# rbuler/multimodal-isic

Hardware: AMD Instinct MI355X
Metric: bags/sec (train step) @ 64x224x224 patches/bag (higher is better)
Workload: dtype bf16; 1 GPU; ISIC-shaped attention-MIL: 256 bags x 64x224x224 patches + 128-d radiomics, ResNet-18 encoder, bf16 (BASELINE.json configs[1]); patches_per_bag=64, patch=3x224x224, radiomics_dim=128, parallelism=dp1

## Files before the change

### multimodal-isic_amd/csrc/conv_stem.hip

```cpp
#include <type_traits>

#include "common.h"
#include "pool_grad.h"

namespace {

constexpr int TH = 8, TW = 16;
constexpr int PR = 2 * TH + 5, PC = 40;
constexpr int PROW = PC * 8;
constexpr int WROW = 7 * 64 + 16;
constexpr int CPAD = 72;
constexpr int YROW = 128 + 32;
constexpr int STEM_DW_ELEMS = 64 * 7 * 7 * 3;
constexpr int STEM_WGRAD_BLOCKS = 512;
constexpr int STEM_FWD_BLOCKS = 768;

struct StemArgs {
  const unsigned short* in;
  const unsigned short* w;
  unsigned short* out;
  const unsigned short* dy;
  float* dw;
  double* stat_sum;
  double* stat_sumsq;
  int stat_slots;
  int N, Hin, Win, Hout, Wout, tiles_h, tiles_w, total_tiles;
};

constexpr int PATCH_PER_THREAD = (PR * PC + 255) / 256;
__device__ __forceinline__ void fetch_patch(u32x2 (&r)[PATCH_PER_THREAD], const StemArgs& a, int tile, int tid) {
  const int n = tile / (a.tiles_h * a.tiles_w);
  const int t2 = tile - n * (a.tiles_h * a.tiles_w);
  const int oy0 = (t2 / a.tiles_w) * TH, ox0 = (t2 % a.tiles_w) * TW;
#pragma unroll
  for (int u = 0; u < PATCH_PER_THREAD; ++u) {
    const int idx = tid + 256 * u;
    const int pr = idx / PC, pc = idx - pr * PC;
    const int hi = 2 * oy0 - 3 + pr, wi = 2 * ox0 - 3 + pc;
    u32x2 v = {0u, 0u};
    if (tile < a.total_tiles && idx < PR * PC && hi >= 0 && hi < a.Hin && wi >= 0 && wi < a.Win)
      v = *reinterpret_cast<const u32x2*>(a.in + (((size_t)n * a.Hin + hi) * a.Win + wi) * 4);
    r[u] = v;
  }
}
__device__ __forceinline__ void commit_patch(unsigned char* Ps, const u32x2 (&r)[PATCH_PER_THREAD], int tid) {
#pragma unroll
  for (int u = 0; u < PATCH_PER_THREAD; ++u) {
    const int idx = tid + 256 * u;
    if (idx < PR * PC) {
      const int pr = idx / PC, pc = idx - pr * PC;
      *reinterpret_cast<u32x2*>(Ps + pr * PROW + pc * 8) = r[u];
    }
  }
}

__global__ __launch_bounds__(256) void conv_stem_fwd_kernel(StemArgs a) {
  static_assert(TH * TW * CPAD * 2 >= PR * PROW, "the C tile overlays the patch");
  __shared__ __attribute__((aligned(16))) unsigned char smem[64 * WROW + TH * TW * CPAD * 2];
  unsigned char* Ws = smem;
  unsigned char* Ps = smem + 64 * WROW;
  unsigned short* Cs = reinterpret_cast<unsigned short*>(smem + 64 * WROW);
  const int tid = threadIdx.x, lane = tid & 63, wave = tid >> 6;
  const int fi = lane & 15, fg = lane >> 4;

  for (int idx = tid; idx < 64 * 28; idx += 256) {
    const int co = idx / 28, ch = idx - co * 28;
    *reinterpret_cast<u32x4*>(Ws + co * WROW + ch * 16) = *reinterpret_cast<const u32x4*>(a.w + co * 224 + ch * 8);
  }

  u32x2 pre[PATCH_PER_THREAD];
  fetch_patch(pre, a, blockIdx.x, tid);
  float st_s[4][4], st_q[4][4];
#pragma unroll
  for (int j = 0; j < 4; ++j)
#pragma unroll
    for (int r = 0; r < 4; ++r) { st_s[j][r] = 0.f; st_q[j][r] = 0.f; }
  for (int tile = blockIdx.x; tile < a.total_tiles; tile += gridDim.x) {
    const int n = tile / (a.tiles_h * a.tiles_w);
    const int t2 = tile - n * (a.tiles_h * a.tiles_w);
    const int oy0 = (t2 / a.tiles_w) * TH, ox0 = (t2 % a.tiles_w) * TW;
    lds_barrier();
    commit_patch(Ps, pre, tid);
    lds_barrier();
    fetch_patch(pre, a, tile + gridDim.x, tid);

    f32x4 acc[2][4];
#pragma unroll
    for (int i = 0; i < 2; ++i)
#pragma unroll
      for (int j = 0; j < 4; ++j) acc[i][j] = (f32x4){0.f, 0.f, 0.f, 0.f};
#pragma unroll
    for (int kh = 0; kh < 7; ++kh) {
      bf16x8 af[2], bfr[4];
#pragma unroll
      for (int i = 0; i < 2; ++i) {
        const int oyl = wave * 2 + i;
        af[i] = *reinterpret_cast<const bf16x8*>(Ps + (2 * oyl + kh) * PROW + (2 * fi + 2 * fg) * 8);
      }
#pragma unroll
      for (int j = 0; j < 4; ++j)
        bfr[j] = *reinterpret_cast<const bf16x8*>(Ws + (j * 16 + fi) * WROW + kh * 64 + fg * 16);
#pragma unroll
      for (int i = 0; i < 2; ++i)
#pragma unroll
        for (int j = 0; j < 4; ++j)
          acc[i][j] = __builtin_amdgcn_mfma_f32_16x16x32_bf16(bfr[j], af[i], acc[i][j], 0, 0, 0);
    }
    lds_barrier();
#pragma unroll
    for (int i = 0; i < 2; ++i)
#pragma unroll
      for (int j = 0; j < 4; ++j) {
        const int p = (wave * 2 + i) * 16 + fi;
        u32x2 v;
        v[0] = (unsigned)f32_to_bf16_bits(acc[i][j][0]) | ((unsigned)f32_to_bf16_bits(acc[i][j][1]) << 16);
        v[1] = (unsigned)f32_to_bf16_bits(acc[i][j][2]) | ((unsigned)f32_to_bf16_bits(acc[i][j][3]) << 16);
        *reinterpret_cast<u32x2*>(Cs + p * CPAD + j * 16 + fg * 4) = v;
        if (a.stat_sum) {
          const bool in = (oy0 + wave * 2 + i < a.Hout) && (ox0 + fi < a.Wout);
          const float r0 = in ? __uint_as_float(v[0] << 16) : 0.f, r1 = in ? __uint_as_float(v[0] & 0xFFFF0000u) : 0.f;
          const float r2 = in ? __uint_as_float(v[1] << 16) : 0.f, r3 = in ? __uint_as_float(v[1] & 0xFFFF0000u) : 0.f;
          st_s[j][0] += r0; st_q[j][0] += r0 * r0;
          st_s[j][1] += r1; st_q[j][1] += r1 * r1;
          st_s[j][2] += r2; st_q[j][2] += r2 * r2;
          st_s[j][3] += r3; st_q[j][3] += r3 * r3;
        }
      }
    lds_barrier();
    for (int idx = tid; idx < TH * TW * 8; idx += 256) {
      const int p = idx >> 3, ch = idx & 7;
      const int oy = oy0 + (p >> 4), ox = ox0 + (p & 15);
      if (oy < a.Hout && ox < a.Wout)
        __builtin_nontemporal_store(*reinterpret_cast<const u32x4*>(Cs + p * CPAD + ch * 8),
                                    reinterpret_cast<u32x4*>(a.out + (((size_t)n * a.Hout + oy) * a.Wout + ox) * 64 + ch * 8));
    }
  }
  if (a.stat_sum) {
    __shared__ float stat_red[2][4][64];
    lds_barrier();
#pragma unroll
    for (int j = 0; j < 4; ++j)
#pragma unroll
      for (int r = 0; r < 4; ++r) {
        float sv = st_s[j][r], qv = st_q[j][r];
#pragma unroll
        for (int o = 8; o > 0; o >>= 1) { sv += __shfl_xor(sv, o, 16); qv += __shfl_xor(qv, o, 16); }
        if (fi == 0) { stat_red[0][wave][j * 16 + fg * 4 + r] = sv; stat_red[1][wave][j * 16 + fg * 4 + r] = qv; }
      }
    lds_barrier();
    if (tid < 128) {
      const int c = tid & 63, w = tid >> 6;
      const float t = (stat_red[w][0][c] + stat_red[w][1][c]) + (stat_red[w][2][c] + stat_red[w][3][c]);
      const size_t slot = (size_t)(blockIdx.x % a.stat_slots) * 64 + c;
      atomicAdd((w == 0 ? a.stat_sum : a.stat_sumsq) + slot, (double)t);
    }
  }
}

__global__ __launch_bounds__(256) void conv_stem_wgrad_kernel(StemArgs a) {
  __shared__ __attribute__((aligned(16))) unsigned char smem[PR * PROW + TH * TW * YROW];
  unsigned char* Ps = smem;
  unsigned char* Ys = smem + PR * PROW;
  const int tid = threadIdx.x, lane = tid & 63, wave = tid >> 6;
  const int fg = lane >> 4, fi = lane & 15, fq = fi >> 2, fp = fi & 3;
  typedef __attribute__((address_space(3))) s16x4* lds_s16x4;

  f32x4 acc[4][4];
#pragma unroll
  for (int i = 0; i < 4; ++i)
#pragma unroll
    for (int j = 0; j < 4; ++j) acc[i][j] = (f32x4){0.f, 0.f, 0.f, 0.f};

  u32x2 pre[PATCH_PER_THREAD];
  u32x4 prey[4];
  auto fetch_dy = [&](int tile) {
    const int n = tile / (a.tiles_h * a.tiles_w);
    const int t2 = tile - n * (a.tiles_h * a.tiles_w);
    const int oy0 = (t2 / a.tiles_w) * TH, ox0 = (t2 % a.tiles_w) * TW;
#pragma unroll
    for (int u = 0; u < 4; ++u) {
      const int idx = tid + 256 * u;
      const int p = idx >> 3, ch = idx & 7;
      const int oy = oy0 + (p >> 4), ox = ox0 + (p & 15);
      u32x4 v = {0u, 0u, 0u, 0u};
      if (tile < a.total_tiles && oy < a.Hout && ox < a.Wout)
        v = *reinterpret_cast<const u32x4*>(a.dy + (((size_t)n * a.Hout + oy) * a.Wout + ox) * 64 + ch * 8);
      prey[u] = v;
    }
  };
  fetch_patch(pre, a, blockIdx.x, tid);
  fetch_dy(blockIdx.x);
  for (int tile = blockIdx.x; tile < a.total_tiles; tile += gridDim.x) {
    lds_barrier();
    commit_patch(Ps, pre, tid);
#pragma unroll
    for (int u = 0; u < 4; ++u) {
      const int idx = tid + 256 * u;
      *reinterpret_cast<u32x4*>(Ys + (idx >> 3) * YROW + (idx & 7) * 16) = prey[u];
    }
    lds_barrier();
    fetch_patch(pre, a, tile + gridDim.x, tid);
    fetch_dy(tile + gridDim.x);
#pragma unroll
    for (int ks = 0; ks < 4; ++ks) {
      const int k1 = ks * 32 + 8 * fg + fq, k2 = k1 + 4;
      bf16x8 af[4], bfr[4];
#pragma unroll
      for (int i = 0; i < 4; ++i) {
        const s16x4 lo = __builtin_amdgcn_ds_read_tr16_b64_v4i16((lds_s16x4)(Ys + k1 * YROW + (i * 16 + 4 * fp) * 2));
        const s16x4 hi = __builtin_amdgcn_ds_read_tr16_b64_v4i16((lds_s16x4)(Ys + k2 * YROW + (i * 16 + 4 * fp) * 2));
        s16x8_t t; t.lo = lo; t.hi = hi;
        af[i] = __builtin_bit_cast(bf16x8, t);
      }
#pragma unroll
      for (int j = 0; j < 4; ++j) {
        const int nt = wave + 4 * j;
        const int kh = nt >> 1, half = nt & 1;
        const int khc = kh > 6 ? 6 : kh;
        const unsigned char* p1 = Ps + (2 * (k1 >> 4) + khc) * PROW + (2 * (k1 & 15) + half * 4 + fp) * 8;
        const unsigned char* p2 = Ps + (2 * (k2 >> 4) + khc) * PROW + (2 * (k2 & 15) + half * 4 + fp) * 8;
        const s16x4 lo = __builtin_amdgcn_ds_read_tr16_b64_v4i16((lds_s16x4)p1);
        const s16x4 hi = __builtin_amdgcn_ds_read_tr16_b64_v4i16((lds_s16x4)p2);
        s16x8_t t; t.lo = lo; t.hi = hi;
        bfr[j] = __builtin_bit_cast(bf16x8, t);
      }
#pragma unroll
      for (int i = 0; i < 4; ++i)
#pragma unroll
        for (int j = 0; j < 4; ++j)
          acc[i][j] = __builtin_amdgcn_mfma_f32_16x16x32_bf16(af[i], bfr[j], acc[i][j], 0, 0, 0);
    }
  }
#pragma unroll
  for (int i = 0; i < 4; ++i)
#pragma unroll
    for (int j = 0; j < 4; ++j) {
      const int nt = wave + 4 * j;
      if (nt >= 14) continue;
      const int kh = nt >> 1, kw = (nt & 1) * 4 + (fi >> 2), c = fi & 3;
      if (kw >= 7 || c >= 3) continue;
#pragma unroll
      for (int r = 0; r < 4; ++r) {
        const int co = i * 16 + fg * 4 + r;
        a.dw[(size_t)blockIdx.x * STEM_DW_ELEMS + ((co * 7 + kh) * 7 + kw) * 3 + c] = acc[i][j][r];
      }
    }
}

struct StemBnArgs {
  StemArgs s;
  const unsigned short* y0;
  const unsigned char* argmax;
  const unsigned short* gp;
  const float* mean; const float* rstd; const float* gamma; const float* scale; const float* shift;
  const double* dgamma; const double* dbeta;
  float* dgamma_f32; float* dbeta_f32;
  int Hp, Wp;
};

__global__ __launch_bounds__(256, 2) void conv_stem_wgrad_bn_kernel(StemBnArgs b) {
  const StemArgs& a = b.s;
  __shared__ __attribute__((aligned(16))) unsigned char smem[PR * PROW + TH * TW * YROW];
  __shared__ __attribute__((aligned(16))) float cst[5][64];
  unsigned char* Ps = smem;
  unsigned char* Ys = smem + PR * PROW;
  const int tid = threadIdx.x, lane = tid & 63, wave = tid >> 6;
  const int fg = lane >> 4, fi = lane & 15, fq = fi >> 2, fp = fi & 3;
  typedef __attribute__((address_space(3))) s16x4* lds_s16x4;
  const isic_pool::PoolGeom geom{a.Hout, a.Wout, 64, b.Hp, b.Wp};

  if (tid < 64) {
    const float inv_rows = 1.f / (float)((int64_t)a.N * a.Hout * a.Wout);
    const float rs = b.rstd[tid], mu = b.mean[tid], k1 = b.gamma[tid] * rs;
    const float k2 = (float)b.dbeta[tid] * inv_rows, k3 = (float)b.dgamma[tid] * inv_rows;
    cst[0][tid] = k1; cst[1][tid] = -k1 * k3 * rs; cst[2][tid] = k1 * (k3 * rs * mu - k2);
    cst[3][tid] = b.scale[tid]; cst[4][tid] = b.shift[tid];
    if (blockIdx.x == 0 && b.dgamma_f32) {
      b.dgamma_f32[tid] += (float)b.dgamma[tid];
      b.dbeta_f32[tid] += (float)b.dbeta[tid];
    }
  }

  f32x4 acc[4][4];
#pragma unroll
  for (int i = 0; i < 4; ++i)
#pragma unroll
    for (int j = 0; j < 4; ++j) acc[i][j] = (f32x4){0.f, 0.f, 0.f, 0.f};

  const int cg = tid & 7, bl = tid >> 3, al = bl >> 3, bw = bl & 7;
  u32x2 pre[PATCH_PER_THREAD];
  u32x4 xr[4];
  isic_pool::Windows win;
  auto fetch_dy = [&](int tile) {
    const int tc = tile < a.total_tiles ? tile : a.total_tiles - 1;
    const int n = tc / (a.tiles_h * a.tiles_w);
    const int t2 = tc - n * (a.tiles_h * a.tiles_w);
    const int oy0 = (t2 / a.tiles_w) * TH, ox0 = (t2 % a.tiles_w) * TW;
    const int ga = (oy0 >> 1) + al, gb = (ox0 >> 1) + bw;
#pragma unroll
    for (int p = 0; p < 4; ++p) {
      const int hi = min(2 * ga + (p >> 1), a.Hout - 1), wi = min(2 * gb + (p & 1), a.Wout - 1);
      xr[p] = *reinterpret_cast<const u32x4*>(b.y0 + (((size_t)n * a.Hout + hi) * a.Wout + wi) * 64 + cg * 8);
    }
    isic_pool::load_windows(win, b.argmax, b.gp, geom, n, min(ga, b.Hp - 1), min(gb, b.Wp - 1), cg);
  };
  auto commit_dy = [&](int tile) {
    const int n = tile / (a.tiles_h * a.tiles_w);
    const int t2 = tile - n * (a.tiles_h * a.tiles_w);
    const int oy0 = (t2 / a.tiles_w) * TH, ox0 = (t2 % a.tiles_w) * TW;
    const int ga = (oy0 >> 1) + al, gb = (ox0 >> 1) + bw;
    const bool inside = (oy0 + TH <= a.Hout) && (ox0 + TW <= a.Wout);
    auto half = [&](auto HC) {
      constexpr int H_ = decltype(HC)::value;
      float g[4][4];
      isic_pool::windows_to_grad4<H_>(win, geom, ga, gb, g);
      const int c0 = cg * 8 + H_ * 4;
      const f32x4 kA = *reinterpret_cast<const f32x4*>(&cst[0][c0]), kB = *reinterpret_cast<const f32x4*>(&cst[1][c0]);
      const f32x4 kD = *reinterpret_cast<const f32x4*>(&cst[2][c0]), sc = *reinterpret_cast<const f32x4*>(&cst[3][c0]);
      const f32x4 sh = *reinterpret_cast<const f32x4*>(&cst[4][c0]);
#pragma unroll
      for (int p = 0; p < 4; ++p) {
        const int oyl = 2 * al + (p >> 1), oxl = 2 * bw + (p & 1);
        const bool in = inside || ((oy0 + oyl < a.Hout) && (ox0 + oxl < a.Wout));
        const unsigned lo = xr[p][2 * H_], hi = xr[p][2 * H_ + 1];
        const float xv[4] = {__uint_as_float(lo << 16), __uint_as_float(lo & 0xFFFF0000u), __uint_as_float(hi << 16),
                             __uint_as_float(hi & 0xFFFF0000u)};
        float o[4];
#pragma unroll
        for (int j = 0; j < 4; ++j) {
          const float dz = (xv[j] * sc[j] + sh[j] > 0.f) ? g[p][j] : 0.f;
          o[j] = kA[j] * dz + (kB[j] * xv[j] + kD[j]);
          if (!inside) o[j] = in ? o[j] : 0.f;
        }
        u32x2 v;
        v[0] = (unsigned)f32_to_bf16_bits(o[0]) | ((unsigned)f32_to_bf16_bits(o[1]) << 16);
        v[1] = (unsigned)f32_to_bf16_bits(o[2]) | ((unsigned)f32_to_bf16_bits(o[3]) << 16);
        *reinterpret_cast<u32x2*>(Ys + (oyl * TW + oxl) * YROW + cg * 16 + H_ * 8) = v;
      }
    };
    half(std::integral_constant<int, 0>{});
    __builtin_amdgcn_sched_barrier(0);
    half(std::integral_constant<int, 1>{});
  };
  __syncthreads();
  fetch_patch(pre, a, blockIdx.x, tid);
  fetch_dy(blockIdx.x);
  for (int tile = blockIdx.x; tile < a.total_tiles; tile += gridDim.x) {
    lds_barrier();
    commit_patch(Ps, pre, tid);
    commit_dy(tile);
    lds_barrier();
    fetch_patch(pre, a, tile + gridDim.x, tid);
    fetch_dy(tile + gridDim.x);
#pragma unroll
    for (int ks = 0; ks < 4; ++ks) {
      const int k1 = ks * 32 + 8 * fg + fq, k2 = k1 + 4;
      bf16x8 af[4], bfr[4];
#pragma unroll
      for (int i = 0; i < 4; ++i) {
        const s16x4 lo = __builtin_amdgcn_ds_read_tr16_b64_v4i16((lds_s16x4)(Ys + k1 * YROW + (i * 16 + 4 * fp) * 2));
        const s16x4 hi = __builtin_amdgcn_ds_read_tr16_b64_v4i16((lds_s16x4)(Ys + k2 * YROW + (i * 16 + 4 * fp) * 2));
        s16x8_t t; t.lo = lo; t.hi = hi;
        af[i] = __builtin_bit_cast(bf16x8, t);
      }
#pragma unroll
      for (int j = 0; j < 4; ++j) {
        const int nt = wave + 4 * j;
        const int kh = nt >> 1, half = nt & 1;
        const int khc = kh > 6 ? 6 : kh;
        const unsigned char* p1 = Ps + (2 * (k1 >> 4) + khc) * PROW + (2 * (k1 & 15) + half * 4 + fp) * 8;
        const unsigned char* p2 = Ps + (2 * (k2 >> 4) + khc) * PROW + (2 * (k2 & 15) + half * 4 + fp) * 8;
        const s16x4 lo = __builtin_amdgcn_ds_read_tr16_b64_v4i16((lds_s16x4)p1);
        const s16x4 hi = __builtin_amdgcn_ds_read_tr16_b64_v4i16((lds_s16x4)p2);
        s16x8_t t; t.lo = lo; t.hi = hi;
        bfr[j] = __builtin_bit_cast(bf16x8, t);
      }
#pragma unroll
      for (int i = 0; i < 4; ++i)
#pragma unroll
        for (int j = 0; j < 4; ++j)
          acc[i][j] = __builtin_amdgcn_mfma_f32_16x16x32_bf16(af[i], bfr[j], acc[i][j], 0, 0, 0);
    }
  }
#pragma unroll
  for (int i = 0; i < 4; ++i)
#pragma unroll
    for (int j = 0; j < 4; ++j) {
      const int nt = wave + 4 * j;
      if (nt >= 14) continue;
      const int kh = nt >> 1, kw = (nt & 1) * 4 + (fi >> 2), c = fi & 3;
      if (kw >= 7 || c >= 3) continue;
#pragma unroll
      for (int r = 0; r < 4; ++r) {
        const int co = i * 16 + fg * 4 + r;
        a.dw[(size_t)blockIdx.x * STEM_DW_ELEMS + ((co * 7 + kh) * 7 + kw) * 3 + c] = acc[i][j][r];
      }
    }
}

__global__ __launch_bounds__(256) void stem_wgrad_reduce_kernel(const float* __restrict__ partial, float* __restrict__ dw,
                                                                 int nparts) {
  const int g = threadIdx.x & 15;
  const int e = blockIdx.x * 16 + (threadIdx.x >> 4);
  float v = 0.f;
  if (e < STEM_DW_ELEMS)
    for (int s = g; s < nparts; s += 16) v += partial[(size_t)s * STEM_DW_ELEMS + e];
#pragma unroll
  for (int o = 8; o > 0; o >>= 1) v += __shfl_xor(v, o, 16);
  if (e < STEM_DW_ELEMS && g == 0) dw[e] += v;
}

__global__ void stem_pack_kernel(const float* __restrict__ w, unsigned short* __restrict__ ws) {
  const int idx = blockIdx.x * blockDim.x + threadIdx.x;
  if (idx >= 64 * 7 * 8 * 4) return;
  const int c = idx & 3, kw = (idx >> 2) & 7, kh = (idx >> 5) % 7, co = idx / 224;
  float v = 0.f;
  if (c < 3 && kw < 7) v = w[((co * 7 + kh) * 7 + kw) * 3 + c];
  ws[idx] = f32_to_bf16_bits(v);
}

int stem_args(StemArgs& a, int N, int Hin, int Win, int Hout, int Wout) {
  if (Hout != (Hin + 6 - 7) / 2 + 1 || Wout != (Win + 6 - 7) / 2 + 1) return ISIC_ERR_BAD_ARG;
  a.N = N; a.Hin = Hin; a.Win = Win; a.Hout = Hout; a.Wout = Wout;
  a.tiles_h = ceil_div(Hout, TH); a.tiles_w = ceil_div(Wout, TW);
  const int64_t tt = (int64_t)N * a.tiles_h * a.tiles_w;
  if (tt > 0x7FFFFFFFLL) return ISIC_ERR_UNSUPPORTED;
  a.total_tiles = (int)tt;
  return ISIC_OK;
}

}

extern "C" {

int isic_conv_stem_fwd_bf16(const uint16_t* in_nhwc4, const uint16_t* w_stem, uint16_t* out, int N, int Hin, int Win,
                            int Hout, int Wout, void* stream) {
  return isic_conv_stem_fwd_stats_bf16(in_nhwc4, w_stem, out, N, Hin, Win, Hout, Wout, nullptr, nullptr, 0, stream);
}

int isic_conv_stem_fwd_stats_bf16(const uint16_t* in_nhwc4, const uint16_t* w_stem, uint16_t* out, int N, int Hin,
                                  int Win, int Hout, int Wout, double* stat_sum, double* stat_sumsq, int stat_slots,
                                  void* stream) {
  ISIC_CHECK_ARG(in_nhwc4 && w_stem && out && N > 0 && Hin > 0 && Win > 0);
  ISIC_CHECK_ARG((stat_sum == nullptr) == (stat_sumsq == nullptr));
  ISIC_CHECK_ARG(!stat_sum || stat_slots > 0);
  StemArgs a;
  a.stat_sum = stat_sum; a.stat_sumsq = stat_sumsq; a.stat_slots = stat_slots > 0 ? stat_slots : 1;
  a.in = in_nhwc4; a.w = w_stem; a.out = out; a.dy = nullptr; a.dw = nullptr;
  int rc = stem_args(a, N, Hin, Win, Hout, Wout);
  if (rc != ISIC_OK) return rc;
  const int grid = a.total_tiles < STEM_FWD_BLOCKS ? a.total_tiles : STEM_FWD_BLOCKS;
  hipLaunchKernelGGL(conv_stem_fwd_kernel, dim3(grid), dim3(256), 0, as_stream(stream), a);
  return isic_launch_status();
}

size_t isic_conv_stem_wgrad_workspace_bytes(void) { return (size_t)STEM_WGRAD_BLOCKS * STEM_DW_ELEMS * sizeof(float); }

int isic_conv_stem_wgrad_bf16(const uint16_t* in_nhwc4, const uint16_t* dy, float* dw, int N, int Hin, int Win,
                              int Hout, int Wout, void* workspace, size_t workspace_bytes, void* stream) {
  ISIC_CHECK_ARG(in_nhwc4 && dy && dw && workspace && N > 0 && Hin > 0 && Win > 0);
  if (workspace_bytes < isic_conv_stem_wgrad_workspace_bytes()) return ISIC_ERR_WORKSPACE;
  StemArgs a;
  a.stat_sum = nullptr; a.stat_sumsq = nullptr; a.stat_slots = 1;
  a.in = in_nhwc4; a.w = nullptr; a.out = nullptr; a.dy = dy; a.dw = reinterpret_cast<float*>(workspace);
  int rc = stem_args(a, N, Hin, Win, Hout, Wout);
  if (rc != ISIC_OK) return rc;
  const int grid = a.total_tiles < STEM_WGRAD_BLOCKS ? a.total_tiles : STEM_WGRAD_BLOCKS;
  hipLaunchKernelGGL(conv_stem_wgrad_kernel, dim3(grid), dim3(256), 0, as_stream(stream), a);
  hipLaunchKernelGGL(stem_wgrad_reduce_kernel, dim3(ceil_div(STEM_DW_ELEMS, 16)), dim3(256), 0, as_stream(stream),
                     reinterpret_cast<const float*>(workspace), dw, grid);
  return isic_launch_status();
}

int isic_conv_stem_wgrad_bn_pooled_bf16(const uint16_t* in_nhwc4, const uint16_t* y0, const uint8_t* argmax,
                                        const uint16_t* dy_pooled, const float* mean, const float* rstd,
                                        const float* gamma, const float* scale, const float* shift, const double* dgamma,
                                        const double* dbeta, float* dw, float* dgamma_f32, float* dbeta_f32, int N,
                                        int Hin, int Win, int Hout, int Wout, int Hp, int Wp, void* workspace,
                                        size_t workspace_bytes, void* stream) {
  ISIC_CHECK_ARG(in_nhwc4 && y0 && argmax && dy_pooled && mean && rstd && gamma && scale && shift && dgamma && dbeta && dw);
  ISIC_CHECK_ARG(workspace != nullptr);
  if (workspace_bytes < isic_conv_stem_wgrad_workspace_bytes()) return ISIC_ERR_WORKSPACE;
  ISIC_CHECK_ARG(N > 0 && Hin > 0 && Win > 0 && (dgamma_f32 == nullptr) == (dbeta_f32 == nullptr));
  ISIC_CHECK_ARG(Hp == (Hout + 2 - 3) / 2 + 1 && Wp == (Wout + 2 - 3) / 2 + 1);
  StemBnArgs b;
  StemArgs& a = b.s;
  a.stat_sum = nullptr; a.stat_sumsq = nullptr; a.stat_slots = 1;
  a.in = in_nhwc4; a.w = nullptr; a.out = nullptr; a.dy = nullptr; a.dw = reinterpret_cast<float*>(workspace);
  int rc = stem_args(a, N, Hin, Win, Hout, Wout);
  if (rc != ISIC_OK) return rc;
  b.y0 = y0; b.argmax = argmax; b.gp = dy_pooled; b.mean = mean; b.rstd = rstd; b.gamma = gamma; b.scale = scale;
  b.shift = shift; b.dgamma = dgamma; b.dbeta = dbeta; b.dgamma_f32 = dgamma_f32; b.dbeta_f32 = dbeta_f32;
  b.Hp = Hp; b.Wp = Wp;
  const int grid = a.total_tiles < STEM_WGRAD_BLOCKS ? a.total_tiles : STEM_WGRAD_BLOCKS;
  hipLaunchKernelGGL(conv_stem_wgrad_bn_kernel, dim3(grid), dim3(256), 0, as_stream(stream), b);
  hipLaunchKernelGGL(stem_wgrad_reduce_kernel, dim3(ceil_div(STEM_DW_ELEMS, 16)), dim3(256), 0, as_stream(stream),
                     reinterpret_cast<const float*>(workspace), dw, grid);
  return isic_launch_status();
}

int isic_conv_stem_pack_bf16(const float* w_krsc, uint16_t* w_stem, void* stream) {
  ISIC_CHECK_ARG(w_krsc && w_stem);
  hipLaunchKernelGGL(stem_pack_kernel, dim3(ceil_div(64 * 224, 256)), dim3(256), 0, as_stream(stream), w_krsc, w_stem);
  return isic_launch_status();
}

}
```

Baseline: 915.8 bags/s.

## Interleave next-tile prefetch with BN backward and inline maxpool grad routing

The fused stem wgrad+BN backward kernel now issues the next tile's patch, y0 and pool-window loads between the halves of the current tile's BN-backward commit, rather than after the LDS barrier. The goal is to hide global-load latency behind ALU work. Maxpool gradient routing is inlined with explicit argmax code selection and bf16 rounding. Blocks are also remapped so neighbouring block ids take strided tile ranges, with partial dw indexed to match. The added sched_barriers and live registers may raise register pressure at 2 waves/SIMD.

Result: faster. 928.1 bags/s (median of 6 runs) (+1.3%).

```diff
diff --git a/multimodal-isic_amd/csrc/conv_stem.hip b/multimodal-isic_amd/csrc/conv_stem.hip
--- a/multimodal-isic_amd/csrc/conv_stem.hip
+++ b/multimodal-isic_amd/csrc/conv_stem.hip
@@ -247,6 +247,21 @@
     }
 }
 
+typedef __attribute__((ext_vector_type(2))) float f32x2;
+typedef __attribute__((ext_vector_type(2))) __bf16 bf16x2;
+__device__ __forceinline__ unsigned pack_bf16x2(float lo, float hi) {
+  return __builtin_bit_cast(unsigned, __builtin_convertvector((f32x2){lo, hi}, bf16x2));
+}
+__device__ __forceinline__ float bn_bwd_value(float kA, float kB, float kD, float x, float dz) {
+#pragma clang fp contract(off)
+  return (kB * x + kD) + kA * dz;
+}
+__device__ __forceinline__ void round_bf16_pair(float& x, float& y) {
+  const unsigned v = pack_bf16x2(x, y);
+  x = __uint_as_float(v << 16);
+  y = __uint_as_float(v & 0xFFFF0000u);
+}
+
 struct StemBnArgs {
   StemArgs s;
   const unsigned short* y0;
@@ -287,33 +302,58 @@
 #pragma unroll
     for (int j = 0; j < 4; ++j) acc[i][j] = (f32x4){0.f, 0.f, 0.f, 0.f};
 
+  const int lb = gridDim.x % 8 == 0 ? (blockIdx.x % 8) * (gridDim.x / 8) + blockIdx.x / 8 : blockIdx.x;
   const int cg = tid & 7, bl = tid >> 3, al = bl >> 3, bw = bl & 7;
   u32x2 pre[PATCH_PER_THREAD];
   u32x4 xr[4];
   isic_pool::Windows win;
-  auto fetch_dy = [&](int tile) {
+  struct TileGeo { int n, oy0, ox0, ga, gb; };
+  auto geo = [&](int tile) {
     const int tc = tile < a.total_tiles ? tile : a.total_tiles - 1;
-    const int n = tc / (a.tiles_h * a.tiles_w);
-    const int t2 = tc - n * (a.tiles_h * a.tiles_w);
-    const int oy0 = (t2 / a.tiles_w) * TH, ox0 = (t2 % a.tiles_w) * TW;
-    const int ga = (oy0 >> 1) + al, gb = (ox0 >> 1) + bw;
-#pragma unroll
-    for (int p = 0; p < 4; ++p) {
-      const int hi = min(2 * ga + (p >> 1), a.Hout - 1), wi = min(2 * gb + (p & 1), a.Wout - 1);
-      xr[p] = *reinterpret_cast<const u32x4*>(b.y0 + (((size_t)n * a.Hout + hi) * a.Wout + wi) * 64 + cg * 8);
-    }
-    isic_pool::load_windows(win, b.argmax, b.gp, geom, n, min(ga, b.Hp - 1), min(gb, b.Wp - 1), cg);
+    TileGeo t;
+    t.n = tc / (a.tiles_h * a.tiles_w);
+    const int t2 = tc - t.n * (a.tiles_h * a.tiles_w);
+    t.oy0 = (t2 / a.tiles_w) * TH; t.ox0 = (t2 % a.tiles_w) * TW;
+    t.ga = (t.oy0 >> 1) + al; t.gb = (t.ox0 >> 1) + bw;
+    return t;
+  };
+  auto fetch_y0 = [&](const TileGeo& t, int p) {
+    const int hi = min(2 * t.ga + (p >> 1), a.Hout - 1), wi = min(2 * t.gb + (p & 1), a.Wout - 1);
+    xr[p] = *reinterpret_cast<const u32x4*>(b.y0 + (((size_t)t.n * a.Hout + hi) * a.Wout + wi) * 64 + cg * 8);
+  };
+  auto fetch_windows = [&](const TileGeo& t) {
+    isic_pool::load_windows(win, b.argmax, b.gp, geom, t.n, min(t.ga, b.Hp - 1), min(t.gb, b.Wp - 1), cg);
   };
   auto commit_dy = [&](int tile) {
-    const int n = tile / (a.tiles_h * a.tiles_w);
-    const int t2 = tile - n * (a.tiles_h * a.tiles_w);
-    const int oy0 = (t2 / a.tiles_w) * TH, ox0 = (t2 % a.tiles_w) * TW;
-    const int ga = (oy0 >> 1) + al, gb = (ox0 >> 1) + bw;
-    const bool inside = (oy0 + TH <= a.Hout) && (ox0 + TW <= a.Wout);
-    auto half = [&](auto HC) {
+    const TileGeo t = geo(tile), nx = geo(tile + gridDim.x);
+    const bool live01 = t.gb + 1 < b.Wp, live10 = t.ga + 1 < b.Hp, live11 = live01 && live10;
+    float dz[2][4][4];
+    auto route = [&](auto HC) {
       constexpr int H_ = decltype(HC)::value;
-      float g[4][4];
-      isic_pool::windows_to_grad4<H_>(win, geom, ga, gb, g);
+      const unsigned am[4] = {win.am[0][H_], live01 ? win.am[1][H_] : ~0u, live10 ? win.am[2][H_] : ~0u,
+                              live11 ? win.am[3][H_] : ~0u};
+#pragma unroll
+      for (int j = 0; j < 4; ++j) {
+        float g[4];
+#pragma unroll
+        for (int k = 0; k < 4; ++k) {
+          const unsigned w = win.g[k][2 * H_ + (j >> 1)];
+          g[k] = __uint_as_float((j & 1) ? (w & 0xFFFF0000u) : (w << 16));
+        }
+        g[0] = g[0] + 0.f;
+        auto sel = [&](int k, unsigned code) { return ((am[k] >> (8 * j)) & 0xFFu) == code ? g[k] : 0.f; };
+        dz[H_][0][j] = sel(0, 4);
+        dz[H_][1][j] = sel(0, 5) + sel(1, 3);
+        dz[H_][2][j] = sel(0, 7) + sel(2, 1);
+        dz[H_][3][j] = ((sel(0, 8) + sel(1, 6)) + sel(2, 2)) + sel(3, 0);
+      }
+#pragma unroll
+      for (int j = 0; j < 4; ++j) round_bf16_pair(dz[H_][1][j], dz[H_][2][j]);
+      round_bf16_pair(dz[H_][3][0], dz[H_][3][1]);
+      round_bf16_pair(dz[H_][3][2], dz[H_][3][3]);
+    };
+    auto bn = [&](auto HC) {
+      constexpr int H_ = decltype(HC)::value;
       const int c0 = cg * 8 + H_ * 4;
       const f32x4 kA = *reinterpret_cast<const f32x4*>(&cst[0][c0]), kB = *reinterpret_cast<const f32x4*>(&cst[1][c0]);
       const f32x4 kD = *reinterpret_cast<const f32x4*>(&cst[2][c0]), sc = *reinterpret_cast<const f32x4*>(&cst[3][c0]);
@@ -321,37 +361,49 @@
 #pragma unroll
       for (int p = 0; p < 4; ++p) {
         const int oyl = 2 * al + (p >> 1), oxl = 2 * bw + (p & 1);
-        const bool in = inside || ((oy0 + oyl < a.Hout) && (ox0 + oxl < a.Wout));
+        const bool in = (t.oy0 + oyl < a.Hout) && (t.ox0 + oxl < a.Wout);
         const unsigned lo = xr[p][2 * H_], hi = xr[p][2 * H_ + 1];
         const float xv[4] = {__uint_as_float(lo << 16), __uint_as_float(lo & 0xFFFF0000u), __uint_as_float(hi << 16),
                              __uint_as_float(hi & 0xFFFF0000u)};
         float o[4];
 #pragma unroll
         for (int j = 0; j < 4; ++j) {
-          const float dz = (xv[j] * sc[j] + sh[j] > 0.f) ? g[p][j] : 0.f;
-          o[j] = kA[j] * dz + (kB[j] * xv[j] + kD[j]);
-          if (!inside) o[j] = in ? o[j] : 0.f;
+          const float d = (__builtin_fmaf(xv[j], sc[j], sh[j]) > 0.f) ? dz[H_][p][j] : 0.f;
+          o[j] = bn_bwd_value(kA[j], kB[j], kD[j], xv[j], d);
         }
         u32x2 v;
-        v[0] = (unsigned)f32_to_bf16_bits(o[0]) | ((unsigned)f32_to_bf16_bits(o[1]) << 16);
-        v[1] = (unsigned)f32_to_bf16_bits(o[2]) | ((unsigned)f32_to_bf16_bits(o[3]) << 16);
+        v[0] = in ? pack_bf16x2(o[0], o[1]) : 0u;
+        v[1] = in ? pack_bf16x2(o[2], o[3]) : 0u;
         *reinterpret_cast<u32x2*>(Ys + (oyl * TW + oxl) * YROW + cg * 16 + H_ * 8) = v;
+        if (H_ == 1) {
+          fetch_y0(nx, p);
+          __builtin_amdgcn_sched_barrier(0);
+        }
       }
     };
-    half(std::integral_constant<int, 0>{});
+    route(std::integral_constant<int, 0>{});
+    bn(std::integral_constant<int, 0>{});
     __builtin_amdgcn_sched_barrier(0);
-    half(std::integral_constant<int, 1>{});
+    route(std::integral_constant<int, 1>{});
+    __builtin_amdgcn_sched_barrier(0);
+    fetch_windows(nx);
+    __builtin_amdgcn_sched_barrier(0);
+    bn(std::integral_constant<int, 1>{});
   };
   __syncthreads();
-  fetch_patch(pre, a, blockIdx.x, tid);
-  fetch_dy(blockIdx.x);
-  for (int tile = blockIdx.x; tile < a.total_tiles; tile += gridDim.x) {
+  fetch_patch(pre, a, lb, tid);
+  {
+    const TileGeo t0 = geo(lb);
+    fetch_windows(t0);
+#pragma unroll
+    for (int p = 0; p < 4; ++p) fetch_y0(t0, p);
+  }
+  for (int tile = lb; tile < a.total_tiles; tile += gridDim.x) {
     lds_barrier();
     commit_patch(Ps, pre, tid);
+    fetch_patch(pre, a, tile + gridDim.x, tid);
     commit_dy(tile);
     lds_barrier();
-    fetch_patch(pre, a, tile + gridDim.x, tid);
-    fetch_dy(tile + gridDim.x);
 #pragma unroll
     for (int ks = 0; ks < 4; ++ks) {
       const int k1 = ks * 32 + 8 * fg + fq, k2 = k1 + 4;
@@ -393,7 +445,7 @@
 #pragma unroll
       for (int r = 0; r < 4; ++r) {
         const int co = i * 16 + fg * 4 + r;
-        a.dw[(size_t)blockIdx.x * STEM_DW_ELEMS + ((co * 7 + kh) * 7 + kw) * 3 + c] = acc[i][j][r];
+        a.dw[(size_t)lb * STEM_DW_ELEMS + ((co * 7 + kh) * 7 + kw) * 3 + c] = acc[i][j][r];
       }
     }
 }
```
